# yangao07/LAMSA

Measured on AMD Instinct MI355X. Metric: aligned Gbase/s, 10 kbp ONT-error reads (12%: sub/ins/del 4% each), -T ont2d vs GRCh37-sized stand-in; inputs resident in HBM when the timed region starts (upload excluded: see pcie_inclusive_*), higher is better.
Workload: dtype int32

## Files before the change

lamsa_amd/csrc/hp_align_api.hip:

```cpp
#include <hip/hip_runtime.h>
#include <algorithm>
#include <atomic>
#include <map>
#include <mutex>
#include <stdlib.h>
#include <string.h>
#include <time.h>
#include "hp_phase.h"
#include "hp_handle.h"
#include "hp_hostprep.h"

using namespace hp;

#ifndef HP_WAVES_PER_SIMD
#define HP_WAVES_PER_SIMD 4
#endif
__global__ __launch_bounds__(64, HP_WAVES_PER_SIMD) void k_align_batch(AlignArgs a)
{
    __shared__ int32_t lds[HP_BOTH_LDS_WORDS];
    const int slot = blockIdx.x;
    for (;;) {
        int u = 0;
        if (wv::leader()) u = atomicAdd(a.counter, 1);
        u = wv::uni(u);
// ... 20 lines not shown
        if (wv::leader()) u = atomicAdd(&a.ctl->q_head[0], 1);
        u = wv::uni(u);
        if (u >= a.n_reads) break;
        phase_chain1(a, a.order ? a.order[u] : u, blockIdx.x, (HP_L int32_t *)lds, WORDS, r);
    }
    drain_stamp(a, 0);
}
template <int WORDS, int WPS>
__global__ __launch_bounds__(64, WPS) void k_chain2(const PhaseArgs *ap)
{
    const PhaseArgs &a = *ap;
    constexpr bool ctx_lds = ph_ctx_in_lds(WORDS, WPS);
    __shared__ alignas(16) int32_t lds[WORDS + (ctx_lds ? PH_CTX_BYTES / 4 : 0)];
    ReadCtx &r = *(ctx_lds ? (ReadCtx *)(lds + WORDS) : (ReadCtx *)(a.slab + (size_t)blockIdx.x * a.slab_per_wave));
    for (;;) {
        int u = 0;
        if (wv::leader()) u = atomicAdd(&a.ctl->q_head[2], 1);
        u = wv::uni(u);
        if (u >= a.n_reads) break;
        phase_chain2(a, a.order ? a.order[u] : u, blockIdx.x, (HP_L int32_t *)lds, WORDS, r);
    }
    drain_stamp(a, 2);
}
typedef void (*ChainKernel)(const PhaseArgs *);
struct ChainShape { ChainKernel k1, k2; int lds_words, waves_per_simd; };
static const ChainShape g_chain_shapes[3] = {
    {k_chain1<HP_CHAIN_LDS_WORDS, HP_CHAIN_WAVES_PER_SIMD>, k_chain2<HP_CHAIN_LDS_WORDS, HP_CHAIN_WAVES_PER_SIMD>, HP_CHAIN_LDS_WORDS, HP_CHAIN_WAVES_PER_SIMD},
    {k_chain1<3392, 3>, k_chain2<3392, 3>, 3392, 3},
    {k_chain1<5120, 2>, k_chain2<5120, 2>, 5120, 2},
};
__global__ __launch_bounds__(64, HP_FILL_WAVES_PER_SIMD) void k_fill(const PhaseArgs *ap, int round)
{
    const PhaseArgs &a = *ap;
    __shared__ int32_t lds[HP_LDS_WORDS];
    int n = 0;
    for (int b = 0; b < PH_NBUCKET; ++b) n += a.ctl->bucket_n[round][b];
    n = wv::uni(n);
    for (;;) {
        int g = 0;
        if (wv::leader()) g = atomicAdd(&a.ctl->q_head[1 + 2 * round], 1);
        g = wv::uni(g);
        if (g >= n) break;
        int b = 0;
        while (b < PH_NBUCKET - 1 && g >= a.ctl->bucket_n[round][b]) { g -= a.ctl->bucket_n[round][b]; ++b; }
        const int u = wv::uni(a.bucket_q[((size_t)round * PH_NBUCKET + b) * a.unit_cap + g]);
        phase_fill(a, round, u, blockIdx.x, (HP_L int32_t *)lds);
    }
    drain_stamp(a, 1 + 2 * round);
}
#ifndef HP_FILLDP_WAVES_PER_SIMD
#define HP_FILLDP_WAVES_PER_SIMD 2
#endif
#ifndef HP_LIST_WAVES_PER_SIMD
#define HP_LIST_WAVES_PER_SIMD 4
#endif
__global__ __launch_bounds__(64, HP_LIST_WAVES_PER_SIMD) void k_filllist(const PhaseArgs *ap, int round)
{
    const PhaseArgs &a = *ap;
    int n = 0;
    for (int b = 0; b < PH_NBUCKET; ++b) n += a.ctl->bucket_n[round][b];
    n = wv::uni(n);
    for (;;) {
        int g = 0;
        if (wv::leader()) g = atomicAdd(&a.ctl->q_head[5], 1);
        g = wv::uni(g);
        if (g >= n) break;
        int b = 0;
        while (b < PH_NBUCKET - 1 && g >= a.ctl->bucket_n[round][b]) { g -= a.ctl->bucket_n[round][b]; ++b; }
        const int u = wv::uni(a.bucket_q[((size_t)round * PH_NBUCKET + b) * a.unit_cap + g]);
        phase_filllist(a, round, u, blockIdx.x, (HP_L int32_t *)nullptr);
    }
}
__global__ __launch_bounds__(64, 2) void k_filldp_small(const PhaseArgs *ap, int round)
{
    __shared__ int32_t lds[HP_LJ_LDS_WORDS(HP_LJ_QSMALL)];
    const PhaseArgs &a = *ap;
    int n = 0;
    for (int b = 0; b < LJ_NBUCKET; ++b) n += ((a.ctl->lj_bucket_n[round][b] < a.lj_cap ? a.ctl->lj_bucket_n[round][b] : a.lj_cap) + 63) >> 6;
    n = wv::uni(n);
    for (;;) {
        int g = 0;
        if (wv::leader()) g = atomicAdd(&a.ctl->q_head[6], 1);
        g = wv::uni(g);
        if (g >= n) break;
        int b = 0;
        for (; b < LJ_NBUCKET - 1; ++b) { const int gb = ((a.ctl->lj_bucket_n[round][b] < a.lj_cap ? a.ctl->lj_bucket_n[round][b] : a.lj_cap) + 63) >> 6; if (g < gb) break; g -= gb; }
        phase_filldp(a, round, b, g * 64, blockIdx.x, (HP_L int32_t *)lds, HP_LJ_QSMALL);
    }
}
__global__ __launch_bounds__(64, HP_WJ_WAVES_PER_SIMD) void k_filldp_wave(const PhaseArgs *ap, int round)
{
    __shared__ int32_t lds[HP_WJ_LDS_WORDS];
    const PhaseArgs &a = *ap;
    int n = 0, n_big = 0;
    for (int b = 0; b < WJ_NBUCKET; ++b) { const int k = a.ctl->wj_bucket_n[round][b] < a.wj_cap ? a.ctl->wj_bucket_n[round][b] : a.wj_cap; if (b < WJ_NBIG) n_big += k; else n += k; }
    n = wv::uni(n); n_big = wv::uni(n_big);
    bool own_big = (int)blockIdx.x < a.n_wjb;
    for (;;) {
        int g = 0;
        const bool big = own_big;
        if (wv::leader()) g = atomicAdd(&a.ctl->q_head[big ? 8 : 7], 1);
        g = wv::uni(g);
        if (g >= (big ? n_big : n)) { if (!big) break; own_big = false; continue; }
// ... 739 lines not shown
```

lamsa_amd/csrc/hp_fill.h:

```cpp
#pragma once
#include "hp_split.h"

namespace hp {

#define HP_REC_MAX 64

struct Rec {
    int64_t offset, refend; int32_t chr, nstrand, readend, score, NM; CigV cig;
    int32_t *mm; int32_t n_mm;
};
struct LineRes {
    int line_score, tol_score, tol_NM, cur_res_n;
    int32_t *ev; int ev_cap;
    Rec rec[HP_REC_MAX];
};

HP_FN bool ref_fetch(ReadCtx &r, int chr, int64_t start0, int32_t *len, uint8_t *dst)
{
    HP_T0(tr0_);
    const int32_t clen = r.ref.seq_len[chr - 1];
    if (start0 > clen || start0 < 0) { r.cx.status |= ST_REFEXIT; return false; }
    if (start0 + *len > clen) *len = (int32_t)(clen - start0);
    const int64_t k0 = r.ref.seq_off[chr - 1] + start0;
    const int32_t n = *len;
// ... 27 lines not shown
        WAVE_FOR(l) {
            const int32_t i = b + l;
            if (i < n) { const int64_t k = k0 + i; dst[i] = pac[k >> 2] >> ((~k & 3) << 1) & 3; }
        }
    }
    wv::sync();
    HP_TADD(r.cx, 30, tr0_);
    return true;
}

HP_FN int cig_pushv_known(Ctx &cx, HP_G cig_t *dst, int &vn_io, int cap, int last, const cig_t *c, int n, int c0)
{
    if (n == 0) return last;
    const HP_G cig_t *src = (const HP_G cig_t *)c;
    const int vn = vn_io;
    int j = 0;
    if (vn > 0) {
        if ((last & 0xf) == (c0 & 0xf)) { last = last + ((c0 >> 4) << 4); dst[vn - 1] = last; j = 1; }
        else if (((last & 0xf) == C_I && (c0 & 0xf) == C_S) || ((last & 0xf) == C_S && (c0 & 0xf) == C_I)) { last = (((last >> 4) + (c0 >> 4)) << 4) | C_S; dst[vn - 1] = last; j = 1; }
    }
    const int m = n - j;
    if (vn + m > cap) { cx.status |= ST_OVERFLOW; return last; }
    if (m > 0) {
        wv::Lane<int> w;
        WAVE_FOR(l) { w[l] = 0; }
        for (int b0 = 0; b0 < m; b0 += 64) { WAVE_FOR(l) { const int i = b0 + l; if (i < m) { w[l] = j + i == 0 ? c0 : (int)src[j + i]; dst[vn + i] = w[l]; } } }
        last = wv::bcast(w, (m - 1) & 63);
    }
    vn_io = vn + m;
    wv::sync();
    return last;
}

HP_NOINL bool merge_cigar_full(ReadCtx &r, CigV &c1, int64_t *c1_refend, int *c1_readend, int chr,
                               const cig_t *_c2, int c2_n, int c2_reflen, int c2_readlen)
{
    if (c2_n == 0) return true;
    Ctx &cx = r.cx;
    HP_T0(tmf_);
    const lamsa_hp_para *P = cx.P;
    HP_G cig_t *const c1c = (HP_G cig_t *)wv::uni64((long long)c1.c);
    const int n1_0 = wv::uni(c1.n), c1cap = wv::uni(c1.cap);
    const int64_t refend0 = *c1_refend; const int readend0 = wv::uni(*c1_readend), read_L = wv::uni(r.L);
    const uint8_t *const cur_read = (const uint8_t *)wv::uni64((long long)r.cur_read);
    const HP_G cig_t *g1 = c1c, *g2 = (const HP_G cig_t *)_c2;
    int vn = n1_0;
    wv::Lane<int> T1, T2;
    WAVE_FOR(l) { T1[l] = l < n1_0 ? (int)g1[n1_0 - 1 - l] : 0; T2[l] = l < c2_n ? (int)g2[l] : 0; }
    bool repair = false;
    if (n1_0 > 1) {
        const int t = wv::bcast(T1, 0), h = wv::bcast(T2, 0);
        const int top = t & 0xf, hop = h & 0xf;
        if ((((top == C_I || top == C_D) && (t >> 4) <= 3) && hop != C_S && hop != C_H) ||
            (((hop == C_I || hop == C_D) && (h >> 4) <= 3) && top != C_S && top != C_H)) repair = true;
    }
    if (!repair) cig_pushv_known(cx, c1c, vn, c1cap, wv::bcast(T1, 0), _c2, c2_n, wv::bcast(T2, 0));
    else {
        const size_t mark = arena_mark(cx.tmp);
        int len1, len11 = 0, len2, len21 = 0, len22 = 0, len_dif1 = 0, len_dif2 = 0;
        int b = 0, min_b, ci = 0, left = 1, right = 1;
        const int md = 5;
        int64_t ref_start = 0; int read_start = 0;
        CigV bd; bd.c = nullptr; bd.n = 0; bd.cap = 0;
        int n1 = n1_0;
#define HP_MF_E1(k) ((k) <= 0 ? 0 : (n1_0 - (k) < 64 ? wv::bcast(T1, n1_0 - (k)) : (int)g1[(k) - 1]))
#define HP_MF_E2(k) ((k) >= c2_n ? 0 : ((k) < 64 ? wv::bcast(T2, (k)) : (int)g2[(k)]))
        int e1 = HP_MF_E1(n1), e2 = HP_MF_E2(0);
        int bd_first = 0, bd_last = 0;
        bool ok = true;
        for (;;) {
            if (left) {
                while (n1 >= 1) {
                    const int op = e1 & 0xf, l = e1 >> 4;
                    if (op == C_M && l > md) { e1 -= md << 4; len21 += md; break; }
                    else if (op == C_M) { len21 += l; --n1; e1 = HP_MF_E1(n1); }
                    else if (op == C_I) { len21 += l; len_dif1 -= l; b += l; --n1; e1 = HP_MF_E1(n1); }
// ... 167 lines not shown
    wv::Lane<int> base = adv;
    wv::scan_add_excl(base);
    { wv::Lane<int> h = S; wv::scan_add_excl(h); WAVE_FOR(l) { S[l] += h[l]; } }
    const unsigned long long mb = wv::ballot(big);
    wv::Lane<int> e_of;
    WAVE_FOR(l) { const unsigned long long above = l < 63 ? (mb >> (l + 1)) << (l + 1) : 0ull; e_of[l] = above ? __builtin_ctzll(above) : K - 1; }
    const wv::Lane<int> S_e = wv::gather(S, e_of);
    HP_G cig_t *out = (HP_G cig_t *)fc.c;
    const int B0 = fc.n - 1;
    const int e0 = mb ? __builtin_ctzll(mb) : K - 1;
    const cig_t top_new = top + (cig_t)(wv::bcast(S, e0) << 4);
    wv::Lane<int> adj;
    WAVE_FOR(l) {
        adj[l] = 0;
        if (l == 0) out[B0] = top_new;
        if (big[l]) {
            adj[l] = wl[l] + ((S_e[l] - S[l]) << 4);
            const HP_G cig_t *w = (const HP_G cig_t *)src[l];
            HP_G cig_t *o = out + B0 + base[l];
            for (int t = 1; t < n[l] - 1; ++t) o[t] = w[t];
            o[n[l] - 1] = adj[l];
        }
    }
    top = mb ? (cig_t)wv::bcast(adj, 63 - __builtin_clzll(mb)) : top_new;
    fc.n += n_new;
    ref_end += wv::reduce_sum(rl); re += wv::reduce_sum(ql); r.cs_words += wv::reduce_sum(cw);
    last = seed_at_after_block(g_seed, i, step, nb);
    wv::sync();
    return nb;
}

HP_NOINL bool frag_extend_multi(ReadCtx &r, const FLines &F, int frag, Rec &res)
{
    Ctx &cx = r.cx;
    const lamsa_hp_para *P = cx.P;
    const int32_t *seed = F.fr_seed + F.fr_seed_off[frag];
    const int seed_n = F.fr_seed_off[frag + 1] - F.fr_seed_off[frag];
    const int strand = r.h_strand[seed[0]], chr = r.h_chr[seed[0]];
    const size_t mark = arena_mark(cx.tmp);
    CigV fc;
    int cap = 0;
    {   const HP_G int32_t *g_seed = (const HP_G int32_t *)seed;
        for (int b0 = 0; b0 < seed_n; b0 += 64) { wv::Lane<int> c; WAVE_FOR(l) { c[l] = b0 + l < seed_n ? (int)r.h_cig_n[g_seed[b0 + l]] : 0; } cap += wv::reduce_sum(c); }
        cap += seed_n * (2 * iabs(P->seed_step) + 64);
    }
    if (!cig_alloc(cx, fc, cap + 16)) return false;
    int i, rs, re, last;
    if (strand == 1) { i = seed_n - 1; last = seed[i]; rs = (sid(r, r.n_seed[last]) - 1) * P->seed_step + 1; }
    else { i = 0; last = seed[0]; rs = r.last_len + (sid(r, r.n_seed[last]) - 1) * P->seed_step + 1; }
    re = rs - 1 + P->seed_len;
    cig_pushv(cx, fc, r.cig + r.h_cig_off[last], r.h_cig_n[last]); r.cs_words += r.h_cig_n[last];
    const int64_t ref_start = r.h_pos[last];
    int64_t ref_end = r.h_pos[last] + P->seed_len - 1 + r.h_len_dif[last];
    const int step = strand == 1 ? -1 : 1;
    bool ok = true;
    i += step;
    while (i >= 0 && i < seed_n && ok) {
        const int left = step == 1 ? seed_n - i : i + 1;
        if (left >= HP_FRAG_BLOCK_MIN && fc.n > 0) {
            cig_t top = ((const HP_G cig_t *)fc.c)[fc.n - 1];
            const int took = frag_steps_block(r, F, frag, i, step, left, fc, ref_end, re, last, top);
            if (took) { HP_STAT(24); i += step * took; continue; }
        }
        const int one_by_one = left < 32 ? left : 32;
        HP_STAT(25);
        for (int t = 0; t < one_by_one && ok; ++t) { ok = frag_step(r, F, frag, i, chr, fc, ref_end, re, last); i += step; }
    }
    if (ok) ok = merge_cigar(r, res.cig, &res.refend, &res.readend, chr, fc.c, fc.n, (int)(ref_end - ref_start + 1), re - rs + 1);
    arena_release(cx.tmp, mark);
    return ok && !(cx.status & (ST_REFEXIT | ST_OVERFLOW));
}

HP_INL bool frag_extend(ReadCtx &r, const FLines &F, int frag, Rec &res)
{
    const int o0 = F.fr_seed_off[frag], o1 = F.fr_seed_off[frag + 1];
    if (o1 - o0 != 1) return frag_extend_multi(r, F, frag, res);
    const lamsa_hp_para *P = r.cx.P;
    const int s = F.fr_seed[o0];
    r.cs_words += r.h_cig_n[s];
    const bool ok = merge_cigar(r, res.cig, &res.refend, &res.readend, r.h_chr[s], r.cig + r.h_cig_off[s], r.h_cig_n[s],
                                P->seed_len + r.h_len_dif[s], P->seed_len);
    return ok && !(r.cx.status & (ST_REFEXIT | ST_OVERFLOW));
}

struct SplitGeo {
    const uint8_t *qp; int64_t at1_off, at2_off; int at1_ld, at1_chr, at2_chr, did, s_qlen, dis, match_dis;
    const int32_t *jt; const int32_t *jarena;
};

HP_NOINL bool split_sv(ReadCtx &r, const SplitGeo &g, Rec &res)
{
    Ctx &cx = r.cx;
    const lamsa_hp_para *P = cx.P;
    const int hash_len = P->hash_len, s_qlen = g.s_qlen, dis = g.dis;
    const uint8_t *qp = g.qp;
    const int64_t at1_off = g.at1_off, at2_off = g.at2_off;
    const int at1_ld = g.at1_ld, at1_chr = g.at1_chr, at2_chr = g.at2_chr;
    const int gh0 = hash_len * P->match;
    const size_t mark = arena_mark(cx.tmp);
    int s_tlen = 0;
    int32_t tl;
    CigV sc;
    bool ok = true;
    if (dis > g.match_dis) {
        s_tlen = s_qlen + dis; tl = s_tlen;
        uint8_t *tb = (uint8_t *)arena_alloc(cx, (size_t)(s_tlen > 0 ? s_tlen : 0) + 16);
        ok = tb && cig_alloc(cx, sc, s_qlen + s_tlen + 64) && ref_fetch(r, at1_chr, at1_off + P->seed_len + at1_ld - 1, &tl, tb);
        if (ok) {
            s_tlen = tl;
            if (s_qlen < hash_len) ksw_bi_extend(cx, s_qlen, seq_fwd(qp), s_tlen, seq_fwd(tb), gh0, gh0, sc);
            else split_indel_map(cx, sc, qp, s_qlen, tb, s_tlen, 0);
        }
    } else {
        s_tlen = s_qlen + dis;
        if (s_tlen < 2 * P->hash_step) {
            int32_t _s_tlen = s_qlen + hash_len;
            int lqe, lte, rqe, rte;
            uint8_t *tb1 = (uint8_t *)arena_alloc(cx, (size_t)_s_tlen + 16), *tb2 = (uint8_t *)arena_alloc(cx, (size_t)_s_tlen + 16);
            CigV lc, rcg;
            ok = tb1 && tb2 && cig_alloc(cx, sc, 2 * (s_qlen + _s_tlen) + 64) && cig_alloc(cx, lc, s_qlen + _s_tlen + 8) && cig_alloc(cx, rcg, s_qlen + _s_tlen + 8);
            ok = ok && ref_fetch(r, at1_chr, at1_off + P->seed_len + at1_ld - 1, &_s_tlen, tb1);
            if (ok) {
                ksw_extend(cx, s_qlen, seq_fwd(qp), _s_tlen, seq_fwd(tb1), P->band_w, gh0, &lqe, &lte, &lc);
                ok = ref_fetch(r, at2_chr, at2_off - _s_tlen - 1, &_s_tlen, tb2);
            }
            if (ok) {
                const Seq rq = seq_rev(qp, s_qlen), rt = seq_rev(tb2, _s_tlen);
                ksw_extend(cx, s_qlen, rq, _s_tlen, rt, P->band_w, gh0, &rqe, &rte, &rcg);
                cig_invert(rcg.c, rcg.n);
                sw_mid_fix(cx, sc, lc.c, lc.n, rcg.c, rcg.n, s_qlen, rq, lqe, rqe, s_qlen + dis, rt, lte, rte);
            }
        } else {
            s_tlen += 2 * (hash_len - dis); tl = s_tlen;
            uint8_t *tb = (uint8_t *)arena_alloc(cx, (size_t)s_tlen + 16);
            ok = tb && cig_alloc(cx, sc, s_qlen + s_tlen + 64) && ref_fetch(r, at1_chr, at1_off + P->seed_len + at1_ld + dis - hash_len - 1, &tl, tb);
            if (ok) {
                s_tlen = tl;
                const int off_dis = (s_tlen != s_qlen - dis + 2 * hash_len) ? 0 : -dis;
                s_tlen = s_qlen + dis;
                if (s_tlen < hash_len) ksw_bi_extend(cx, s_qlen, seq_fwd(qp), s_tlen, seq_fwd(tb + hash_len - dis), gh0, gh0, sc);
                else split_indel_map(cx, sc, qp, s_qlen, tb + hash_len - dis, s_tlen, off_dis);
            }
        }
    }
    if (ok) ok = merge_cigar(r, res.cig, &res.refend, &res.readend, at1_chr, sc.c, sc.n, s_tlen, s_qlen);
    arena_release(cx.tmp, mark);
    return ok && !(cx.status & (ST_REFEXIT | ST_OVERFLOW));
}

HP_NOINL bool split_mismatch(ReadCtx &r, const SplitGeo &g, Rec &res)
{
    Ctx &cx = r.cx;
    const lamsa_hp_para *P = cx.P;
    int s_tlen = g.s_qlen + g.dis;
    if (s_tlen < 0) { cx.status |= ST_REFEXIT; return false; }
    if (g.jt && g.jt[3] && g.jarena) {
        return merge_cigar(r, res.cig, &res.refend, &res.readend, g.at1_chr, g.jarena + g.jt[0], g.jt[1], g.jt[2], g.s_qlen) && !(cx.status & (ST_REFEXIT | ST_OVERFLOW));
    }
    const size_t mark = arena_mark(cx.tmp);
    int32_t tl = s_tlen;
    CigV sc;
    uint8_t *tb = (uint8_t *)arena_alloc(cx, (size_t)s_tlen + 16);
    bool ok = tb && cig_alloc(cx, sc, g.s_qlen + s_tlen + 64) && ref_fetch(r, g.at1_chr, g.at1_off + P->seed_len + g.at1_ld - 1, &tl, tb);
    if (ok) {
        s_tlen = tl;
        ksw_bi_extend(cx, g.s_qlen, seq_fwd(g.qp), s_tlen, seq_fwd(tb), 100, 100, sc);
        ok = merge_cigar(r, res.cig, &res.refend, &res.readend, g.at1_chr, sc.c, sc.n, s_tlen, g.s_qlen);
    }
    arena_release(cx.tmp, mark);
    return ok && !(cx.status & (ST_REFEXIT | ST_OVERFLOW));
}

HP_INL bool split_mapping(ReadCtx &r, const FLines &F, int f1, int f2, Rec &res)
{
    Ctx &cx = r.cx;
    const lamsa_hp_para *P = cx.P;
    const int32_t *sd1 = F.fr_seed + F.fr_seed_off[f1], *sd2 = F.fr_seed + F.fr_seed_off[f2];
    const int n1 = F.fr_seed_off[f1 + 1] - F.fr_seed_off[f1], n2 = F.fr_seed_off[f2 + 1] - F.fr_seed_off[f2];
    int s1, s2;
    if (r.h_strand[sd1[0]] == 1) { s1 = sd1[0]; s2 = sd2[n2 - 1]; }
    else { s1 = sd1[n1 - 1]; s2 = sd2[0]; }
    SplitGeo g;
    g.at1_off = r.h_pos[s1]; g.at2_off = r.h_pos[s2];
    g.at1_ld = r.h_len_dif[s1]; g.at1_chr = r.h_chr[s1]; g.at2_chr = r.h_chr[s2];
// ... 588 lines not shown
```

lamsa_amd/csrc/hp_ksw.h:

```cpp
#pragma once
#include "hp_core.h"

namespace hp {

#define HP_ZSTRIDE(n_col) ((((n_col) + 7) >> 3) << 2)
HP_INL size_t z_cap(const Ctx &cx) { const int w = cx.lds_words - (2 * HP_LDS_CELLS + HP_LDS_CELLS / 4); return w > 0 ? (size_t)w * 4 : 0; }
HP_INL size_t z_cap_pk(const Ctx &cx) { return cx.lds_words > 0 ? (size_t)cx.lds_words * 4 : 0; }
#define HP_ZFITS(n_col, rows) ((size_t)HP_ZSTRIDE(n_col) * (size_t)(rows) <= z_cap(cx))
HP_INL int z_nibble(int dir) { return (dir & 3) | ((dir >> 2) & 1) << 2 | ((dir >> 5) & 1) << 3; }
HP_INL void z_row_clear(HP_L uint8_t *LZ, int row, int n_col) {
    HP_L int *p = (HP_L int *)(LZ + row * HP_ZSTRIDE(n_col));
    const int nd = HP_ZSTRIDE(n_col) >> 2;
    for (int d0 = 0; d0 < nd; d0 += 64) { WAVE_FOR(l) { if (d0 + l < nd) p[d0 + l] = -1; } }
}
HP_INL void z_put(HP_L uint8_t *LZ, int row, int n_col, int c, int dir) {
    HP_L int *p = (HP_L int *)(LZ + row * HP_ZSTRIDE(n_col)) + (c >> 3);
    wv::lds_and(p, (int)~((unsigned)(~z_nibble(dir) & 0xf) << ((c & 7) << 2)));
}

HP_FN void dp_backtrack(Ctx &cx, const HP_L uint8_t *lz, const uint8_t *z, const int32_t *rowb, int n_col, int w, int i, int k, CigV &out, int pk_stride = 0)
{
    pk_stride = wv::uni(pk_stride);
    const bool in_lds = z == nullptr;
    const HP_G uint8_t *gz = (const HP_G uint8_t *)wv::uni64((long long)z);
// ... 1409 lines not shown
    int Sn = qlen - lqe - rqe, Hn = tlen - lte - rte, half = P->split_len / 2;
    if (iabs(Sn) >= half || iabs(Hn) >= half || iabs(Sn - Hn) >= half || tlen < 0 || qlen < 0) {
        cig_pushv(cx, out, lc, ln);
        cig_push0(cx, out, (cig_t)((uint32_t)Sn << 4) | C_S);
        cig_push0(cx, out, (cig_t)((uint32_t)Hn << 4) | C_H);
        cig_pushv(cx, out, rc, rn);
    } else {
        const size_t mark = arena_mark(cx.tmp);
        CigV g;
        if (cig_alloc(cx, g, qlen + tlen + 2)) {
            ksw_global(cx, qlen, q, tlen, t, P->del_gapo, P->del_gape, P->ins_gapo, P->ins_gape, P->band_w, &g);
            cig_pushv(cx, out, g.c, g.n);
        }
        arena_release(cx.tmp, mark);
    }
}

HP_INL bool bi_near_diag(const lamsa_hp_para *P, int qlen, int tlen)
{
#if defined(__HIP_DEVICE_COMPILE__)
    float a = __fmul_rn((float)tlen, P->id_rate);
    float b = __fmul_rn(a, (float)(P->aln_mode & 2));
    float c = __fadd_rn((float)P->split_len, b);
#else
    volatile float a = (float)tlen * P->id_rate;
    volatile float b = a * (float)(P->aln_mode & 2);
    volatile float c = (float)P->split_len + b;
#endif
    return (float)iabs(qlen - tlen) < c;
}

HP_NOINL int ksw_bi_extend(Ctx &cx_, int qlen, Seq q, int tlen, Seq t, int lh0, int rh0, CigV &out_)
{
    Ctx &cx = *(Ctx *)wv::uni64((long long)&cx_);
    CigV &out = *(CigV *)wv::uni64((long long)&out_);
    qlen = wv::uni(qlen); tlen = wv::uni(tlen); lh0 = wv::uni(lh0); rh0 = wv::uni(rh0);
    q.p = (const uint8_t *)wv::uni64((long long)q.p); q.stride = wv::uni(q.stride);
    t.p = (const uint8_t *)wv::uni64((long long)t.p); t.stride = wv::uni(t.stride);
    const lamsa_hp_para *P = (const lamsa_hp_para *)wv::uni64((long long)cx.P);
    out.n = 0;
    if (qlen < 0 || tlen < 0) { cx.status |= ST_REFEXIT; return 0; }
    if (qlen == 0 && lh0 > 0) {
        if (tlen > 0) cig_raw_push(cx, out, (tlen << 4) | C_D);
        return 0;
    }
    HP_T0(tbi0_);
    const size_t mark = arena_mark(cx.tmp);
    int ret = 0, res, lqe, lte, rqe, rte;
    CigV L, R;
    if (!cig_alloc(cx, L, qlen + tlen + 4) || !cig_alloc(cx, R, qlen + tlen + 4)) { arena_release(cx.tmp, mark); return 0; }
    L.c = (cig_t *)wv::uni64((long long)L.c); R.c = (cig_t *)wv::uni64((long long)R.c); L.cap = wv::uni(L.cap); R.cap = wv::uni(R.cap);
    const int band_w = wv::uni(P->band_w);
    const int w = iabs(qlen - tlen) + 3 > band_w ? iabs(qlen - tlen) + 3 : band_w;
    res = ksw_extend_c(cx, qlen, q, tlen, t, w, lh0, &lqe, &lte, &L);
    res = wv::uni(res); lqe = wv::uni(lqe); lte = wv::uni(lte);
    HP_T0(tbi1_);
    if (res < 2) {
        cig_pushv(cx, out, L.c, L.n);
        cig_push1(cx, out, res == 0 ? ((tlen - lte) << 4) | C_D : ((qlen - lqe) << 4) | C_I);
    } else if (bi_near_diag(P, qlen, tlen) && ((lqe << 1 > qlen) || (lte << 1 > tlen))) {
        ksw_global(cx, qlen, q, tlen, t, P->del_gapo, P->del_gape, P->ins_gapo, P->ins_gape, P->band_w, &out);
    } else {
        res = ksw_extend_r(cx, qlen, q, tlen, t, w, rh0, &rqe, &rte, &R);
        res = wv::uni(res); rqe = wv::uni(rqe); rte = wv::uni(rte);
        if (res < 2) {
            cig_push1(cx, R, res == 0 ? ((tlen - rte) << 4) | C_D : ((qlen - rqe) << 4) | C_I);
// ... 18 lines not shown
```

lamsa_amd/csrc/hp_phase.h:

```cpp
#pragma once
#include "hp_align.h"
#include "hp_lanedp.h"
#include "hp_wavejob.h"

namespace hp {

struct RdMeta {
    int64_t fl_off[2];
    int32_t fl_n[2], fl_tot[2], fl_nfrag[2];
    int32_t unit_base[2];
    int32_t status;
    int32_t tbases;
    int32_t cells, pairs;
    int32_t cs_words, pad_;
};

struct UnitRec {
    int32_t read, line;
    int64_t out_off;
    int32_t out_len, n_reg;
    int32_t pad[2];
};

enum { PH_NBUCKET = 8, PH_REG_WORDS = 10 };
// ... 77 lines not shown
        const int bucket = PH_NBUCKET - 1 - b;
        UnitRec &U = a.units[(size_t)round * a.unit_cap + base + j];
        U.read = rd; U.line = j; U.out_off = 0; U.out_len = 0; U.n_reg = 0;
        int at = 0;
        if (wv::leader()) at = atomicAdd(&a.ctl->bucket_n[round][bucket], 1);
        at = wv::uni(at);
        a.bucket_q[((size_t)round * PH_NBUCKET + bucket) * a.unit_cap + at] = base + j;
    }
}

HP_INL void pers_bind(ReadCtx &r, const PhaseArgs &a, int rd)
{
    const int64_t pb = r.hb + rd;
    r.nd = a.g_nd + pb; r.n_seed = a.g_nseed + pb;
    r.srt = a.g_sidx + 2 * pb; r.rnk = a.g_sidx + 2 * pb + (r.H + 1);
}

#ifdef HP_PROF
#define PH_T0() const long long ph_t0_ = wv::clock()
#define PH_TADD(k) do { if (r.prof) r.prof[k] += wv::clock() - ph_t0_; } while (0)
#define PH_TMID(k, v) do { if (r.prof) { const long long now_ = wv::clock(); r.prof[k] += now_ - v; v = now_; } } while (0)
#else
#define PH_T0() do { } while (0)
#define PH_TADD(k) do { } while (0)
#define PH_TMID(k, v) do { } while (0)
#endif

enum { PH_CTX_BYTES = 512 };
static_assert(sizeof(ReadCtx) <= PH_CTX_BYTES, "the read context must fit its per-wave block");
constexpr bool ph_ctx_in_lds(int words, int waves_per_simd)
{
    return 4 * waves_per_simd * (((size_t)words * 4 + PH_CTX_BYTES + 511) / 512 * 512) <= 160 * 1024;
}
struct ChainOut { FLines F; FlStore fs; };

HP_NOINL void phase_chain1(const PhaseArgs &a, int rd, int wave_slot, HP_L int32_t *lds, int lds_words, ReadCtx &r)
{
#ifdef HP_PROF
    long long ph_t_ = wv::clock();
#endif
    if (a.in.read_skip && a.in.read_skip[rd]) { if (wv::leader()) atomicOr(&a.meta[rd].status, ST_UNSUPPORTED); return; }
    read_bind(r, a.P, a.ref, a.in, rd, a.slab + (size_t)wave_slot * a.slab_per_wave + PH_CTX_BYTES, a.slab_per_wave - PH_CTX_BYTES, lds, a.prof, lds_words);
    pers_bind(r, a, rd);
    Ctx &cx = r.cx;
    const int H = r.H, c = H + 1;
    ChainOut *co = (ChainOut *)arena_alloc(cx, sizeof(ChainOut));
    int32_t *nm = (int32_t *)arena_alloc(cx, sizeof(int32_t) * 10 * (size_t)c);
    const size_t sort_mark = arena_mark(cx.tmp);
    uint64_t *sort_work = (uint64_t *)arena_alloc(cx, sizeof(uint64_t) * (size_t)c);
    if (co && nm && sort_work) {
        int32_t *sidx = a.g_sidx + 2 * (r.hb + rd);
        { HP_T0(t_sort_);
        sort_read_hits(r.h_pos, r.h_chr, r.h_strand, H, sidx, sidx + c, sort_work, (HP_L uint64_t *)lds, lds_words / 2, a.sort_pb, a.sort_cb);
        HP_TADD(cx, 46, t_sort_); }
        arena_release(cx.tmp, sort_mark);
        aux_bind(r, nm);
        nodes_fill(r);
        PH_TMID(0, ph_t_);
        FLines &F = co->F;
        FlStore &fs = co->fs; fs.base = a.fl_base; fs.cap = a.fl_cap; fs.cursor = &a.ctl->fl_cursor; fs.got_off = 0; fs.got_tot = 0;
#if defined(HP_CHAIN_STOP) && HP_CHAIN_STOP == 0
        const bool ok1 = true; F.n = 0; F.nfrag = 0;
#else
        const bool ok1 = chain_first(r, F, &fs);
#endif
        PH_TMID(1, ph_t_);
        if (ok1 && F.n > 0) units_push(a, r, rd, 0, F, fs);
        else if (!ok1 && !(cx.status & (ST_REFEXIT | ST_OVERFLOW))) cx.status |= ST_OVERFLOW;
    }
    meta_flag(a, rd, r);
}

HP_FN void phase_chain1(const PhaseArgs &a, int rd, int wave_slot, HP_L int32_t *lds, int lds_words = HP_CHAIN_LDS_WORDS)
{
    ReadCtx r;
    phase_chain1(a, rd, wave_slot, lds, lds_words, r);
}

HP_NOINL void phase_fill(const PhaseArgs &a, int round, int u, int wave_slot, HP_L int32_t *lds)
{
    UnitRec &U = a.units[(size_t)round * a.unit_cap + u];
    const int rd = U.read, line = U.line;
    RdMeta &M = a.meta[rd];
    if (*(volatile int32_t *)&M.status & ST_DEAD) return;
    PH_T0();
    ReadCtx r;
    read_bind(r, a.P, a.ref, a.in, rd, a.slab + (size_t)wave_slot * a.slab_fill, a.slab_fill, lds, a.prof, HP_LDS_WORDS);
    pers_bind(r, a, rd);
    Ctx &cx = r.cx;
    FLines F;
    F.n = M.fl_n[round]; F.nfrag = M.fl_nfrag[round];
    flines_bind(F, a.fl_base + M.fl_off[round], F.n, M.fl_tot[round]);
    F.jarena = a.job_base;
    const int cur_cap = 2 * r.L + 512;
    const bool tags = (a.in.tags & LAMSA_HP_TAG_MISMATCHES) != 0;
    const int out_cap = 64 + 12 * r.L + PH_REG_WORDS * HP_REC_MAX + (tags ? line_ev_words(r.L) : 0);
    OutBuf o; o.n = 0; o.cap = out_cap;
    o.w = (int32_t *)arena_alloc(cx, sizeof(int32_t) * (size_t)out_cap);
    r.rc_read = (uint8_t *)arena_alloc(cx, (size_t)r.L + 16);
    LineRes *la = (LineRes *)arena_alloc(cx, sizeof(LineRes));
    cig_t *cur_buf = (cig_t *)arena_alloc(cx, sizeof(cig_t) * (size_t)cur_cap);
    cig_t *rec_buf = (cig_t *)arena_alloc(cx, sizeof(cig_t) * (size_t)(cur_cap + 4 * HP_REC_MAX));
    int32_t *ev = tags ? (int32_t *)arena_alloc(cx, sizeof(int32_t) * (size_t)line_ev_cap(r.L)) : nullptr;
    int n_reg = 0;
    if (o.w && r.rc_read && la && cur_buf && rec_buf && (ev || !tags)) {
        la->ev = ev; la->ev_cap = tags ? line_ev_cap(r.L) : 0;
        const bool ok = fill_line(r, F, line, *la, cur_buf, cur_cap, rec_buf, cur_cap + 4 * HP_REC_MAX);
        if (!ok && !(cx.status & (ST_REFEXIT | ST_OVERFLOW))) cx.status |= ST_OVERFLOW;
        if (ok) {
            out_line(cx, o, *la);
            if (round == 0 && la->tol_score >= 0) {
                Regs G; G.n = 0; G.m = 0;
                const size_t mark = arena_mark(cx.tmp);
                G.beg = (int32_t *)arena_alloc(cx, sizeof(int32_t) * 2 * HP_REC_MAX); G.end = G.beg ? G.beg + HP_REC_MAX : nullptr;
                G.rb = (RegB *)arena_alloc(cx, sizeof(RegB) * 2 * HP_REC_MAX); G.re = G.rb ? G.rb + HP_REC_MAX : nullptr;
                if (G.beg && G.rb) {
                    for (int k = 0; k <= la->cur_res_n; ++k) regs_push(r, G, HP_REC_MAX, la->rec[k]);
                    for (int k = 0; k < G.n; ++k) {
                        out_put(cx, o, G.beg[k]); out_put(cx, o, G.end[k]);
                        out_put(cx, o, G.rb[k].is_rev); out_put(cx, o, G.rb[k].chr); out_put(cx, o, (int32_t)(G.rb[k].pos & 0xffffffffll)); out_put(cx, o, (int32_t)(G.rb[k].pos >> 32));
                        out_put(cx, o, G.re[k].is_rev); out_put(cx, o, G.re[k].chr); out_put(cx, o, (int32_t)(G.re[k].pos & 0xffffffffll)); out_put(cx, o, (int32_t)(G.re[k].pos >> 32));
                    }
                    n_reg = G.n;
                }
                arena_release(cx.tmp, mark);
            }
        }
    }
    if (!(cx.status & (ST_REFEXIT | ST_OVERFLOW))) {
        unsigned long long off = 0;
        if (wv::leader()) off = atomicAdd(&a.ctl->line_cursor, (unsigned long long)o.n);
        off = (unsigned long long)wv::uni64((long long)off);
        if ((int64_t)(off + (unsigned long long)o.n) <= a.line_cap) {
            HP_G int32_t *dst = (HP_G int32_t *)(a.line_base + off);
            const HP_G int32_t *src = (const HP_G int32_t *)o.w;
            wv::sync();
            for (int b = 0; b < o.n; b += 64) { WAVE_FOR(l) { const int i = b + l; if (i < o.n) dst[i] = src[i]; } }
            U.out_off = (int64_t)off; U.out_len = o.n; U.n_reg = n_reg;
        } else cx.status |= ST_OVERFLOW;
    }
    PH_TADD(round == 0 ? 2 : 4);
    meta_flag(a, rd, r);
}


struct LjRec { int64_t qaddr, tk, slot; int32_t rd; uint16_t tlen; uint8_t qlen; int8_t type_comp; };
enum { LJ_NCLS = HP_LJ_QSMALL / 16, LJ_NBUCKET = 2 * LJ_NCLS };
HP_INL int lj_bucket_of(int type, int qlen)
{
    const int cls = (qlen > 0 ? qlen - 1 : 0) >> 4;
    return (type == 1 ? 0 : LJ_NCLS) + (LJ_NCLS - 1 - cls);
}

struct EndGeo { int s, read_start, read_len, chr; int64_t start0; int32_t ref_len; };
HP_INL bool end_geo(const ReadCtx &r, const FLines &F, int line, int strand, bool head, EndGeo &G)
{
    const lamsa_hp_para *P = r.cx.P;
    const int f0 = F.frag_off[line], fl = F.frag_off[line + 1] - 1;
    const int lb = strand == 1 ? F.left_bound[line] : r.seed_all + 1 - F.right_bound[line];
    const int rb = strand == 1 ? F.right_bound[line] : r.seed_all + 1 - F.left_bound[line];
    const int s_first = F.fr_seed[F.fr_seed_off[f0]], s_last = F.fr_seed[F.fr_seed_off[fl + 1] - 1];
    int64_t ref_start;
    if (head) {
        if (strand == 1) {
            G.s = s_last;
            const int id = sid(r, r.n_seed[G.s]);
            if (id == 1) return false;
            G.read_len = (lb == 0 ? 0 : P->seed_inv) + (id - lb - 1) * P->seed_step;
            G.read_start = lb == 0 ? 0 : lb * P->seed_step - P->seed_inv;
        } else {
            G.s = s_first;
            G.read_len = (lb == 0 ? r.last_len : P->seed_inv) + (sid(r, r.n_seed[G.s]) - 1 - lb) * P->seed_step;
            G.read_start = lb == 0 ? 0 : r.last_len + lb * P->seed_step - P->seed_inv;
        }
        if (G.read_len <= 0) return false;
        G.ref_len = G.read_len + P->hash_step * 2;
        ref_start = r.h_pos[G.s] - G.ref_len;
        if (ref_start < 1) { ref_start = 1; G.ref_len = (int32_t)(r.h_pos[G.s] - 1); }
    } else {
        if (strand == 1) {
            G.s = s_first;
            const int id = sid(r, r.n_seed[G.s]);
            G.read_start = id * P->seed_step - P->seed_inv;
            G.read_len = (rb == r.seed_all + 1 ? r.last_len : P->seed_inv) + (rb - 1 - id) * P->seed_step;
        } else {
            G.s = s_last;
            const int id = sid(r, r.n_seed[G.s]);
            if (id == r.seed_all) return false;
            G.read_start = id * P->seed_step - P->seed_inv + r.last_len;
            G.read_len = (rb == r.seed_all + 1 ? 0 : P->seed_inv) + (rb - 1 - id) * P->seed_step;
        }
        if (G.read_len <= 0) return false;
        G.ref_len = G.read_len + P->hash_step * 2;
        ref_start = r.h_pos[G.s] + P->seed_len + r.h_len_dif[G.s];
    }
    G.chr = r.h_chr[G.s];
    G.start0 = ref_start - 1;
    const int32_t clen = r.ref.seq_len[G.chr - 1];
    if (G.start0 > clen || G.start0 < 0) return false;
    if (G.start0 + G.ref_len > clen) G.ref_len = (int32_t)(clen - G.start0);
    return G.ref_len > 0 && G.read_start >= 0 && G.read_start + G.read_len <= r.L;
}

HP_NOINL void phase_filllist(const PhaseArgs &a, int round, int u, int wave_slot, HP_L int32_t *lds)
{
    UnitRec &U = a.units[(size_t)round * a.unit_cap + u];
    const int rd = U.read, line = U.line;
    RdMeta &M = a.meta[rd];
    if (*(volatile int32_t *)&M.status & ST_DEAD) return;
    ReadCtx r;
    read_bind(r, a.P, a.ref, a.in, rd, a.slab + (size_t)wave_slot * a.slab_fill, a.slab_fill, lds, a.prof, 0);
    pers_bind(r, a, rd);
    const lamsa_hp_para *P = r.cx.P;
    const bool lane_ok = lj_params_ok(P) && a.lj_cap > 0, wave_ok = a.wj_cap > 0;
    if (!lane_ok && !wave_ok) return;
    FLines F;
    F.n = M.fl_n[round]; F.nfrag = M.fl_nfrag[round];
    flines_bind(F, a.fl_base + M.fl_off[round], F.n, M.fl_tot[round]);
    const int f0 = F.frag_off[line], nfr = F.frag_off[line + 1] - f0;
    const int p0 = F.fr_seed_off[f0], np = F.fr_seed_off[f0 + nfr] - p0;
    const int strand = r.h_strand[F.fr_seed[p0]];
    const int n_junc = (nfr - 1) + np, n_cand = n_junc + 2;
    r.flip = strand != 1;
    const int64_t rbase = a.in.read_off[rd];
    long long tb = 0;
    int32_t *frag_of = (int32_t *)arena_alloc(r.cx, sizeof(int32_t) * (size_t)(np + 1));
    if (!frag_of) { r.flip = false; return; }
    {
        HP_G int32_t *g_fo = (HP_G int32_t *)frag_of;
        const HP_G int32_t *g_so = (const HP_G int32_t *)F.fr_seed_off;
        for (int b0 = 0; b0 < nfr; b0 += 64) { WAVE_FOR(l) { const int f = f0 + b0 + l; if (b0 + l < nfr) { for (int q = g_so[f]; q < g_so[f + 1]; ++q) g_fo[q - p0] = f; } } }
        wv::sync();
    }
    long long *cand = (long long *)arena_alloc(r.cx, sizeof(long long) * 4 * (size_t)(n_cand + 64));
    if (!cand) { r.flip = false; return; }
    int n_lb[LJ_NBUCKET], n_wb[WJ_NBUCKET];
#pragma unroll
    for (int b = 0; b < LJ_NBUCKET; ++b) n_lb[b] = 0;
#pragma unroll
    for (int b = 0; b < WJ_NBUCKET; ++b) n_wb[b] = 0;
    for (int c0 = 0; c0 < n_cand; c0 += 64) {
        wv::Lane<int> ty, qo, ql, tl, qrev; wv::Lane<long long> tk, sl;
        WAVE_FOR(l) {
// ... 128 lines not shown
                }
            }
            if (mw) {
                wv::Lane<int> at, bk;
                WAVE_FOR(l) {
                    at[l] = base_w + __builtin_popcountll(mw & ((1ull << l) - 1)); bk[l] = -1;
                    if (big[l]) {
                        const int type = ty[l] & 15;
                        WjRec &J = a.wjobs[at[l]];
                        const int back = qrev[l] ? 1 : 0, comp = strand == 1 ? 0 : 1;
                        J.qaddr = strand == 1 ? rbase + qo[l] : rbase + (r.L - 1 - qo[l]);
                        J.tk = tk[l]; J.slot = sl[l]; J.rd = rd; J.qlen = ql[l]; J.tlen = tl[l];
                        J.type_comp = type | (comp << 4) | ((back ^ comp) << 5) | (back << 6);
                        bk[l] = wj_bucket_of(P, type, ql[l], tl[l], wj_need(P, type, ql[l], tl[l]) > (long long)a.slab_wj);
                    }
                }
                base_w += __builtin_popcountll(mw);
#pragma unroll
                for (int b = 0; b < WJ_NBUCKET; ++b) {
                    wv::Lane<int> inb;
                    WAVE_FOR(l) inb[l] = bk[l] == b;
                    const unsigned long long mb = wv::ballot(inb);
                    if (!mb) continue;
                    WAVE_FOR(l) { if (inb[l]) a.wj_bucket[(size_t)b * a.wj_cap + pos_wb[b] + __builtin_popcountll(mb & ((1ull << l) - 1))] = at[l]; }
                    pos_wb[b] += __builtin_popcountll(mb);
                }
            }
            tb += wv::reduce_sum(tbl);
        }
    }
    r.flip = false;
    r.t_bases = tb;
    meta_flag(a, rd, r);
}

HP_INL void phase_filldp(const PhaseArgs &a, int round, int bucket, int off, int wave_slot, HP_L int32_t *lds, int qcap)
{
    const lamsa_hp_para *P = &a.P;
    const int n_in = a.ctl->lj_bucket_n[round][bucket] < a.lj_cap ? a.ctl->lj_bucket_n[round][bucket] : a.lj_cap;
    const int cnt = n_in - off < 64 ? n_in - off : 64;
    char *slab = a.slab + (size_t)wave_slot * a.slab_fill;
    cig_t *cbuf = (cig_t *)slab;
    uint8_t *zbuf = (uint8_t *)(slab + sizeof(cig_t) * 3 * HP_LJ_CIG * 64);
    if (sizeof(cig_t) * 3 * HP_LJ_CIG * 64 + (size_t)qcap * HP_LJ_TSMALL * 64 + 64 > a.slab_fill) return;
    const int32_t *bq = a.lj_bucket + (size_t)bucket * a.lj_cap + off;
    wv::Lane<int> nw, rdl, cel; wv::Lane<long long> slotl;
    wv::sync();
    WAVE_FOR(l) {
        nw[l] = 0; rdl[l] = -1; cel[l] = 0; slotl[l] = 0;
        if (l < cnt && bq[l] >= 0) {
            const LjRec R = a.ljobs[bq[l]];
            LaneJob J;
            const int comp = (R.type_comp >> 4) & 1, type = R.type_comp & 15;
            J.q = (const HP_G uint8_t *)(a.in.read_seq + R.qaddr); J.qs = comp ? -1 : 1; J.qcomp = comp; J.qlen = R.qlen; J.pac = (const HP_G uint8_t *)a.ref.pac; J.tk = R.tk; J.ts = 1; J.tlen = R.tlen;
            J.z = (HP_G uint8_t *)zbuf; J.zl = l; J.zs = qcap; J.cells = 0; J.row = lds + l; J.qrow = (HP_L uint8_t *)(lds + (qcap + 2) * 64) + l; J.rev = 0;
            lj_stage_query(J);
            LCig out, Lc, Rc;
            out.c = cbuf + (size_t)l * 3 * HP_LJ_CIG; out.n = 0; Lc.c = out.c + HP_LJ_CIG; Lc.n = 0; Rc.c = Lc.c + HP_LJ_CIG; Rc.n = 0;
            if (type == 1) lj_bi_extend(P, J, 100, 100, Lc, Rc, out);
            else lj_global(P, J, P->del_gapo, P->del_gape, P->ins_gapo, P->ins_gape, P->band_w, &out);
            nw[l] = out.n; rdl[l] = R.rd; cel[l] = (int)J.cells; slotl[l] = R.slot | ((long long)R.tlen << 48);
        }
    }
    wv::Lane<int> pre = nw;
    wv::scan_add_excl(pre);
    const int total = wv::reduce_sum(nw);
// ... 163 lines not shown
```

lamsa_amd/csrc/hp_split.h:

```cpp
#pragma once
#include "hp_chain.h"
#include "hp_ksw.h"

namespace hp {

#define HP_HASH_SV_PEN 2
#define HP_HASH_MAX_HITS 50

HP_INL unsigned kmer_code(const uint8_t *s, int hash_len)
{
    unsigned v = 0;
    for (int i = 0; i < hash_len; ++i) { unsigned b = s[i]; v = v << 2 | (b > 3 ? 2u : b); }
    return v;
}

struct HCtx {
    const lamsa_hp_para *P; int ref_len, read_len, ref_offset;
    int32_t *nstart, *len_a;
    int32_t *h_from, *h_read_i, *h_offset, *h_score, *h_node_n, *h_slot; int8_t *h_match, *h_dp;
};

HP_FN int hnode_dis(const HCtx &c, int a_i, int a_offset, int b_i, int b_offset)
{
    const int hash_len = c.P->hash_len, hash_step = c.P->hash_step;
// ... 112 lines not shown
        }
        arena_release(cx.tmp, mark);
        for (int i = 0; i < node_i / 2; ++i) { int t = line[i]; line[i] = line[node_i - 1 - i]; line[node_i - 1 - i] = t; }
        return node_i;
    }
    for (int i = 2; i <= hash_seed_n; ++i)
        for (int k = c.nstart[i], e = c.nstart[i] + c.len_a[i]; k < e; ++k)
            if (c.h_dp[k] == MULTI_FLAG) { HP_STAT(13); hdp_update(c, k, 1, MULTI_FLAG); }
    hdp_update(c, tail, 1, MULTI_FLAG);
    node_i = c.h_node_n[tail] - 1;
    int cur = c.h_from[tail];
    while (hslot_of(c, cur) != 0) {
        if (node_i < 0 || cur < 0) { cx.status |= ST_REFEXIT; return 0; }
        line[node_i--] = cur;
        cur = c.h_from[cur];
    }
    if (node_i >= 0) { cx.status |= ST_REFEXIT; return 0; }
    return c.h_node_n[tail];
}

HP_FN int indel_cigar(Ctx &cx, int ref_left, int read_left, int ref_right, int read_right, cig_t *cg, int *clen, int split_len, int *split_flag)
{
    const int dlen = ref_left - ref_right + 1, ilen = read_left - read_right + 1;
    if (dlen < 0 && ilen < 0) { cx.status |= ST_REFEXIT; *clen = 0; return 0; }
    const int len = ilen - dlen;
    if (len > 0) { *clen = 1; cg[0] = (len << 4) + C_D; if (len >= split_len) *split_flag |= 2; }
    else if (len < 0) { *clen = 1; cg[0] = ((0 - len) << 4) + C_I; if (-len >= split_len) *split_flag |= 2; }
    else *clen = 0;
    return dlen > ilen ? dlen : ilen;
}

HP_NOINL int split_indel_map(Ctx &cx, CigV &out, const uint8_t *read_seq, int read_len, const uint8_t *ref_seq, int ref_len, int ref_offset)
{
    const lamsa_hp_para *P = cx.P;
    const int hash_len = P->hash_len, hash_step = P->hash_step, split_len = P->split_pen;
    int res = 0;
    out.n = 0;
    if (read_len < hash_len) { cx.status |= ST_REFEXIT; return 0; }
    const size_t mark = arena_mark(cx.tmp);
    const int n_codes = ref_len - hash_len + 1 > 0 ? ref_len - hash_len + 1 : 0;
    const int hash_seed_n = (read_len - hash_len) / hash_step + 1;
    uint32_t *rcode = (uint32_t *)arena_alloc(cx, sizeof(uint32_t) * (size_t)(n_codes + 1));
    int32_t *nstart = (int32_t *)arena_alloc(cx, sizeof(int32_t) * (size_t)(hash_seed_n + 3));
    int32_t *len_a = (int32_t *)arena_alloc(cx, sizeof(int32_t) * (size_t)(hash_seed_n + 3));
    int32_t *line = (int32_t *)arena_alloc(cx, sizeof(int32_t) * (size_t)(hash_seed_n + 2));
    if (!rcode || !nstart || !len_a || !line) { arena_release(cx.tmp, mark); return 0; }
    for (int b0 = 0; b0 < n_codes; b0 += 64) {
        WAVE_FOR(l) { int i = b0 + l; if (i < n_codes) rcode[i] = kmer_code(ref_seq + i, hash_len); }
    }
    wv::sync();
    int nn = 1;
    len_a[0] = 1;
    for (int s = 1; s <= hash_seed_n; ++s) {
        const unsigned qc = kmer_code(read_seq + (s - 1) * hash_step, hash_len);
        int cnt = 0;
        for (int b0 = 0; b0 < n_codes && cnt <= HP_HASH_MAX_HITS; b0 += 64) {
            wv::Lane<int> eq;
            WAVE_FOR(l) { int i = b0 + l; eq[l] = (i < n_codes && rcode[i] == qc); }
            cnt += __builtin_popcountll(wv::ballot(eq));
        }
        len_a[s] = cnt > HP_HASH_MAX_HITS ? 0 : cnt;
        nn += len_a[s];
    }
    len_a[hash_seed_n + 1] = 1; ++nn;
    const int node_cap = nn + 1;
    int32_t *nm = (int32_t *)arena_alloc(cx, sizeof(int32_t) * 6 * (size_t)node_cap);
// ... 118 lines not shown
```

Measured before the change: 3.814.

## Place fill-phase ReadCtx in LDS and move fill locals to the arena

The fill and fill-list kernels now reserve an LDS block per wave for the ReadCtx and pass it into phase_fill/phase_filllist, replacing the per-thread stack (scratch) copy. Large fill locals (FLines, OutBuf, Regs) move into the per-wave arena, and merge_cigar_full arguments are made wave-uniform so they can sit in scalar registers. The aim is to cut scratch-memory traffic and vector register pressure. In exchange the fill kernel uses more LDS per block, which may limit occupancy, and some HP_STAT counters are added.

```diff
diff --git a/lamsa_amd/csrc/hp_align_api.hip b/lamsa_amd/csrc/hp_align_api.hip
--- a/lamsa_amd/csrc/hp_align_api.hip
+++ b/lamsa_amd/csrc/hp_align_api.hip
@@ -76,7 +76,8 @@
 __global__ __launch_bounds__(64, HP_FILL_WAVES_PER_SIMD) void k_fill(const PhaseArgs *ap, int round)
 {
     const PhaseArgs &a = *ap;
-    __shared__ int32_t lds[HP_LDS_WORDS];
+    __shared__ alignas(16) int32_t lds[HP_LDS_WORDS + PH_CTX_BYTES / 4];
+    ReadCtx &r = *(ReadCtx *)(lds + HP_LDS_WORDS);
     int n = 0;
     for (int b = 0; b < PH_NBUCKET; ++b) n += a.ctl->bucket_n[round][b];
     n = wv::uni(n);
@@ -88,7 +89,7 @@
         int b = 0;
         while (b < PH_NBUCKET - 1 && g >= a.ctl->bucket_n[round][b]) { g -= a.ctl->bucket_n[round][b]; ++b; }
         const int u = wv::uni(a.bucket_q[((size_t)round * PH_NBUCKET + b) * a.unit_cap + g]);
-        phase_fill(a, round, u, blockIdx.x, (HP_L int32_t *)lds);
+        phase_fill(a, round, u, blockIdx.x, (HP_L int32_t *)lds, r);
     }
     drain_stamp(a, 1 + 2 * round);
 }
@@ -101,6 +102,8 @@
 __global__ __launch_bounds__(64, HP_LIST_WAVES_PER_SIMD) void k_filllist(const PhaseArgs *ap, int round)
 {
     const PhaseArgs &a = *ap;
+    __shared__ alignas(16) int32_t lds[PH_CTX_BYTES / 4];
+    ReadCtx &r = *(ReadCtx *)lds;
     int n = 0;
     for (int b = 0; b < PH_NBUCKET; ++b) n += a.ctl->bucket_n[round][b];
     n = wv::uni(n);
@@ -112,7 +115,7 @@
         int b = 0;
         while (b < PH_NBUCKET - 1 && g >= a.ctl->bucket_n[round][b]) { g -= a.ctl->bucket_n[round][b]; ++b; }
         const int u = wv::uni(a.bucket_q[((size_t)round * PH_NBUCKET + b) * a.unit_cap + g]);
-        phase_filllist(a, round, u, blockIdx.x, (HP_L int32_t *)nullptr);
+        phase_filllist(a, round, u, blockIdx.x, (HP_L int32_t *)lds, r);
     }
 }
 __global__ __launch_bounds__(64, 2) void k_filldp_small(const PhaseArgs *ap, int round)
diff --git a/lamsa_amd/csrc/hp_fill.h b/lamsa_amd/csrc/hp_fill.h
--- a/lamsa_amd/csrc/hp_fill.h
+++ b/lamsa_amd/csrc/hp_fill.h
@@ -83,16 +83,22 @@
     return last;
 }
 
-HP_NOINL bool merge_cigar_full(ReadCtx &r, CigV &c1, int64_t *c1_refend, int *c1_readend, int chr,
+HP_NOINL bool merge_cigar_full(ReadCtx &r_, CigV &c1_, int64_t *c1_refend, int *c1_readend, int chr,
                                const cig_t *_c2, int c2_n, int c2_reflen, int c2_readlen)
 {
     if (c2_n == 0) return true;
+    HP_STAT(26);
+    ReadCtx &r = *(ReadCtx *)wv::uni64((long long)&r_);
+    CigV &c1 = *(CigV *)wv::uni64((long long)&c1_);
+    c1_refend = (int64_t *)wv::uni64((long long)c1_refend); c1_readend = (int *)wv::uni64((long long)c1_readend);
+    _c2 = (const cig_t *)wv::uni64((long long)_c2);
+    chr = wv::uni(chr); c2_n = wv::uni(c2_n); c2_reflen = wv::uni(c2_reflen); c2_readlen = wv::uni(c2_readlen);
     Ctx &cx = r.cx;
     HP_T0(tmf_);
-    const lamsa_hp_para *P = cx.P;
+    const lamsa_hp_para *P = (const lamsa_hp_para *)wv::uni64((long long)cx.P);
     HP_G cig_t *const c1c = (HP_G cig_t *)wv::uni64((long long)c1.c);
     const int n1_0 = wv::uni(c1.n), c1cap = wv::uni(c1.cap);
-    const int64_t refend0 = *c1_refend; const int readend0 = wv::uni(*c1_readend), read_L = wv::uni(r.L);
+    const int64_t refend0 = wv::uni64(*c1_refend); const int readend0 = wv::uni(*c1_readend), read_L = wv::uni(r.L);
     const uint8_t *const cur_read = (const uint8_t *)wv::uni64((long long)r.cur_read);
     const HP_G cig_t *g1 = c1c, *g2 = (const HP_G cig_t *)_c2;
     int vn = n1_0;
@@ -326,6 +332,7 @@
 
 HP_NOINL bool frag_extend_multi(ReadCtx &r, const FLines &F, int frag, Rec &res)
 {
+    HP_STAT(27);
     Ctx &cx = r.cx;
     const lamsa_hp_para *P = cx.P;
     const int32_t *seed = F.fr_seed + F.fr_seed_off[frag];
@@ -384,6 +391,7 @@
 
 HP_NOINL bool split_sv(ReadCtx &r, const SplitGeo &g, Rec &res)
 {
+    HP_STAT(28);
     Ctx &cx = r.cx;
     const lamsa_hp_para *P = cx.P;
     const int hash_len = P->hash_len, s_qlen = g.s_qlen, dis = g.dis;
@@ -444,6 +452,7 @@
 
 HP_NOINL bool split_mismatch(ReadCtx &r, const SplitGeo &g, Rec &res)
 {
+    HP_STAT(29);
     Ctx &cx = r.cx;
     const lamsa_hp_para *P = cx.P;
     int s_tlen = g.s_qlen + g.dis;
diff --git a/lamsa_amd/csrc/hp_ksw.h b/lamsa_amd/csrc/hp_ksw.h
--- a/lamsa_amd/csrc/hp_ksw.h
+++ b/lamsa_amd/csrc/hp_ksw.h
@@ -1465,6 +1465,7 @@
 
 HP_NOINL int ksw_bi_extend(Ctx &cx_, int qlen, Seq q, int tlen, Seq t, int lh0, int rh0, CigV &out_)
 {
+    HP_STAT(31);
     Ctx &cx = *(Ctx *)wv::uni64((long long)&cx_);
     CigV &out = *(CigV *)wv::uni64((long long)&out_);
     qlen = wv::uni(qlen); tlen = wv::uni(tlen); lh0 = wv::uni(lh0); rh0 = wv::uni(rh0);
diff --git a/lamsa_amd/csrc/hp_phase.h b/lamsa_amd/csrc/hp_phase.h
--- a/lamsa_amd/csrc/hp_phase.h
+++ b/lamsa_amd/csrc/hp_phase.h
@@ -133,6 +133,8 @@
 {
     return 4 * waves_per_simd * (((size_t)words * 4 + PH_CTX_BYTES + 511) / 512 * 512) <= 160 * 1024;
 }
+static_assert(PH_CTX_BYTES % 512 == 0, "the LDS block of a wave is sized in units of 512 bytes");
+static_assert(28 * (4 * HP_LDS_WORDS + PH_CTX_BYTES) <= 160 * 1024, "DP rows + read context of 7 waves per SIMD must fit the CU's LDS");
 struct ChainOut { FLines F; FlStore fs; };
 
 HP_NOINL void phase_chain1(const PhaseArgs &a, int rd, int wave_slot, HP_L int32_t *lds, int lds_words, ReadCtx &r)
@@ -172,31 +174,46 @@
     meta_flag(a, rd, r);
 }
 
+#ifdef HP_PH_CTX_SHARED
+HP_INL ReadCtx &ph_frame_ctx()
+{
+    alignas(16) static thread_local unsigned char blk[PH_CTX_BYTES];
+    static thread_local bool born = false;
+    if (!born) { for (int i = 0; i < PH_CTX_BYTES; ++i) blk[i] = 0xa5; born = true; }
+    return *reinterpret_cast<ReadCtx *>(blk);
+}
+#define PH_FRAME_CTX(r) ReadCtx &r = ph_frame_ctx()
+#else
+#define PH_FRAME_CTX(r) ReadCtx r##_frame_; ReadCtx &r = r##_frame_
+#endif
 HP_FN void phase_chain1(const PhaseArgs &a, int rd, int wave_slot, HP_L int32_t *lds, int lds_words = HP_CHAIN_LDS_WORDS)
 {
-    ReadCtx r;
+    PH_FRAME_CTX(r);
     phase_chain1(a, rd, wave_slot, lds, lds_words, r);
 }
 
-HP_NOINL void phase_fill(const PhaseArgs &a, int round, int u, int wave_slot, HP_L int32_t *lds)
+struct FillLoc { FLines F; OutBuf o; Regs G; };
+
+HP_NOINL void phase_fill(const PhaseArgs &a, int round, int u, int wave_slot, HP_L int32_t *lds, ReadCtx &r)
 {
     UnitRec &U = a.units[(size_t)round * a.unit_cap + u];
     const int rd = U.read, line = U.line;
     RdMeta &M = a.meta[rd];
     if (*(volatile int32_t *)&M.status & ST_DEAD) return;
     PH_T0();
-    ReadCtx r;
     read_bind(r, a.P, a.ref, a.in, rd, a.slab + (size_t)wave_slot * a.slab_fill, a.slab_fill, lds, a.prof, HP_LDS_WORDS);
     pers_bind(r, a, rd);
     Ctx &cx = r.cx;
-    FLines F;
+    FillLoc *fl = (FillLoc *)arena_alloc(cx, sizeof(FillLoc));
+    if (!fl) { meta_flag(a, rd, r); return; }
+    FLines &F = fl->F;
     F.n = M.fl_n[round]; F.nfrag = M.fl_nfrag[round];
     flines_bind(F, a.fl_base + M.fl_off[round], F.n, M.fl_tot[round]);
     F.jarena = a.job_base;
     const int cur_cap = 2 * r.L + 512;
     const bool tags = (a.in.tags & LAMSA_HP_TAG_MISMATCHES) != 0;
     const int out_cap = 64 + 12 * r.L + PH_REG_WORDS * HP_REC_MAX + (tags ? line_ev_words(r.L) : 0);
-    OutBuf o; o.n = 0; o.cap = out_cap;
+    OutBuf &o = fl->o; o.n = 0; o.cap = out_cap;
     o.w = (int32_t *)arena_alloc(cx, sizeof(int32_t) * (size_t)out_cap);
     r.rc_read = (uint8_t *)arena_alloc(cx, (size_t)r.L + 16);
     LineRes *la = (LineRes *)arena_alloc(cx, sizeof(LineRes));
@@ -211,7 +228,7 @@
         if (ok) {
             out_line(cx, o, *la);
             if (round == 0 && la->tol_score >= 0) {
-                Regs G; G.n = 0; G.m = 0;
+                Regs &G = fl->G; G.n = 0; G.m = 0;
                 const size_t mark = arena_mark(cx.tmp);
                 G.beg = (int32_t *)arena_alloc(cx, sizeof(int32_t) * 2 * HP_REC_MAX); G.end = G.beg ? G.beg + HP_REC_MAX : nullptr;
                 G.rb = (RegB *)arena_alloc(cx, sizeof(RegB) * 2 * HP_REC_MAX); G.re = G.rb ? G.rb + HP_REC_MAX : nullptr;
@@ -244,6 +261,11 @@
     meta_flag(a, rd, r);
 }
 
+HP_FN void phase_fill(const PhaseArgs &a, int round, int u, int wave_slot, HP_L int32_t *lds)
+{
+    PH_FRAME_CTX(r);
+    phase_fill(a, round, u, wave_slot, lds, r);
+}
 
 struct LjRec { int64_t qaddr, tk, slot; int32_t rd; uint16_t tlen; uint8_t qlen; int8_t type_comp; };
 enum { LJ_NCLS = HP_LJ_QSMALL / 16, LJ_NBUCKET = 2 * LJ_NCLS };
@@ -303,13 +325,12 @@
     return G.ref_len > 0 && G.read_start >= 0 && G.read_start + G.read_len <= r.L;
 }
 
-HP_NOINL void phase_filllist(const PhaseArgs &a, int round, int u, int wave_slot, HP_L int32_t *lds)
+HP_NOINL void phase_filllist(const PhaseArgs &a, int round, int u, int wave_slot, HP_L int32_t *lds, ReadCtx &r)
 {
     UnitRec &U = a.units[(size_t)round * a.unit_cap + u];
     const int rd = U.read, line = U.line;
     RdMeta &M = a.meta[rd];
     if (*(volatile int32_t *)&M.status & ST_DEAD) return;
-    ReadCtx r;
     read_bind(r, a.P, a.ref, a.in, rd, a.slab + (size_t)wave_slot * a.slab_fill, a.slab_fill, lds, a.prof, 0);
     pers_bind(r, a, rd);
     const lamsa_hp_para *P = r.cx.P;
@@ -504,6 +525,12 @@
     r.flip = false;
     r.t_bases = tb;
     meta_flag(a, rd, r);
+}
+
+HP_FN void phase_filllist(const PhaseArgs &a, int round, int u, int wave_slot, HP_L int32_t *lds)
+{
+    PH_FRAME_CTX(r);
+    phase_filllist(a, round, u, wave_slot, lds, r);
 }
 
 HP_INL void phase_filldp(const PhaseArgs &a, int round, int bucket, int off, int wave_slot, HP_L int32_t *lds, int qcap)
diff --git a/lamsa_amd/csrc/hp_split.h b/lamsa_amd/csrc/hp_split.h
--- a/lamsa_amd/csrc/hp_split.h
+++ b/lamsa_amd/csrc/hp_split.h
@@ -168,6 +168,7 @@
 
 HP_NOINL int split_indel_map(Ctx &cx, CigV &out, const uint8_t *read_seq, int read_len, const uint8_t *ref_seq, int ref_len, int ref_offset)
 {
+    HP_STAT(30);
     const lamsa_hp_para *P = cx.P;
     const int hash_len = P->hash_len, hash_step = P->hash_step, split_len = P->split_pen;
     int res = 0;
```

Measured after the change: 3.940 (median of 6 runs). +3.3%, better.
